# peterdavidfagan/mujoco_robot_environments

Measured on AMD Instinct MI355X. Metric: env steps/sec (whole node), RearrangementEnv batch=4096 at 1/2/4/8 MI355X, higher is better.
Workload: dtype f32

## Files before the change

### mujoco_robot_environments_amd/csrc/mre_api.cpp

```cpp
#include <hip/hip_runtime.h>

#include <cmath>
#include <cstdio>
#include <cstdlib>
#include <cstring>
#include <string>
#include <algorithm>
#include <vector>

#include "mre_env.h"
#include "mre_launch.h"
#include "mre_model.h"
#include "mre_records.h"

using namespace mre;

static thread_local std::string g_err;
int mre::fail(int code, const std::string& msg) {
  g_err = msg;
  return code;
}

extern "C" const char* mre_last_error(void) { return g_err.c_str(); }

// ... 27 lines not shown
  HIPCHK(hipMalloc(&e->sv_status, N * 4));
  HIPCHK(hipMalloc(&e->sv_converged, N));
  HIPCHK(hipHostMalloc((void**)&e->h_launch_info, mre_env::RING * N * 16, hipHostMallocMapped | hipHostMallocCoherent));
  HIPCHK(hipHostGetDevicePointer((void**)&e->d_launch_info, e->h_launch_info, 0));
  memset(e->h_launch_info, 0xFF, mre_env::RING * N * 16);
  HIPCHK(hipHostMalloc((void**)&e->h_info_last, N * 16, hipHostMallocDefault));
  memset(e->h_info_last, 0xFF, N * 16);
  HIPCHK(hipHostMalloc((void**)&e->h_large_stage, mre_env::NSTAGE * N, hipHostMallocMapped | hipHostMallocCoherent));
  HIPCHK(hipHostGetDevicePointer((void**)&e->d_large_stage, e->h_large_stage, 0));
  memset(e->h_large_stage, 0, mre_env::NSTAGE * N);
  HIPCHK(hipMalloc(&e->d_pending, N));
  HIPCHK(hipMemsetAsync(e->d_pending, 0, N, e->stream));
  HIPCHK(hipMemsetAsync(e->d_large, 0, N, e->stream));
  e->h_large.assign(N, 0); e->h_rerun.assign(N, 0);
  { int rc = sched_create(e); if (rc) return rc; }
  if (const char* fb = getenv("MRE_NO_FALLBACK")) e->fallback = atoi(fb) == 0;
  if (const char* fl = getenv("MRE_FORCE_LARGE")) {
    if (atoi(fl) != 0) {
      e->h_large.assign(N, 1); e->n_large = num_envs;
      HIPCHK(hipMemsetAsync(e->d_large, 1, N, e->stream));
    }
  }
  HIPCHK(hipMemsetAsync(e->status, 0, N * 4, e->stream)); HIPCHK(hipMemsetAsync(e->stats, 0, N * 16, e->stream));
  HIPCHK(hipMemsetAsync(e->grip_closed, 0, N, e->stream)); HIPCHK(hipMemsetAsync(e->osc_target, 0, N * 64, e->stream));
  HIPCHK(hipMemsetAsync(e->sites, 0, N * 64, e->stream));
  std::vector<int> np(N, NPROP);
  std::vector<float> ps(N * NPROP * 3, 0.0155f);
  HIPCHK(hipMemcpy(e->nprops, np.data(), N * 4, hipMemcpyHostToDevice));
  HIPCHK(hipMemcpy(e->prop_size, ps.data(), ps.size() * 4, hipMemcpyHostToDevice));
  e->osc = OscConfig{350.f, 20.f, 500.f, 100.f, 200.f, 30.f, {0.f, -0.785f, 0.f, -2.356f, 0.f, 1.571f, 0.785f},
// ... 552 lines not shown
  DRAIN(e);
  return copy_out(e, w, e->qacc_ws, (size_t)e->N * NVP * 4);
}
extern "C" int mre_set_ctrl(mre_env* e, const float* ctrl) {
  if (!e || !ctrl) return fail(MRE_ERR_ARG, "null");
  DRAIN(e);
  return copy_in(e, e->ctrl, ctrl, (size_t)e->N * NU * 4);
}

static void fill_args(mre_env* e, StepArgs& a) {
  memset(&a, 0, sizeof(a));
  a.M = e->dM; a.N = e->N; a.seq_stride = e->N;
  a.qpos = e->qpos; a.qvel = e->qvel; a.qacc_ws = e->qacc_ws; a.ctrl = e->ctrl; a.qfine = e->qfine;
  a.nprops = e->nprops; a.prop_size = e->prop_size;
  a.control_steps = 1; a.mode = CTRL_HELD;
  a.osc = e->d_osc_env ? e->d_osc_env : e->d_osc; a.osc_stride = e->d_osc_env ? 1 : 0;
  a.osc_target = e->osc_target; a.grip_closed = e->grip_closed;
  a.sites = e->sites; a.status = e->status; a.stats = e->stats; a.nstep = e->nstep;
  a.env_order = e->use_order ? e->order : (e->have_auto_order ? e->auto_order : nullptr);
  a.trace = e->trace; a.trace_nenv = e->trace_nenv; a.trace_max = e->trace_max; a.trace_base = e->trace_pos;
}

extern "C" int mre_step(mre_env* e, int nsubsteps, unsigned flags) {
  if (!e || nsubsteps < 0) return fail(MRE_ERR_ARG, "mre_step: bad argument");
  StepArgs a;
  fill_args(e, a);
  a.nsteps = nsubsteps; a.flags = flags;
  if (nsubsteps > 0) a.sites = nullptr;
  int rc = launch_step(e, a);
  if (rc) return rc;
  if (e->trace) e->trace_pos += nsubsteps;
  return MRE_OK;
}

extern "C" int mre_rollout_ticks(mre_env* e, const float* ctrl_seq, int nticks, int control_steps, unsigned flags,
                                 int ticks_per_launch) {
  if (!e || !ctrl_seq || nticks < 0 || control_steps < 1) return fail(MRE_ERR_ARG, "mre_rollout: bad argument");
  if (!is_device_ptr(ctrl_seq)) return fail(MRE_ERR_ARG, "mre_rollout: ctrl_seq must be a device pointer");
  int per = (ticks_per_launch <= 0 || ticks_per_launch > nticks) ? nticks : ticks_per_launch;
  bool allow_queue = ticks_per_launch >= 2;
  if (ticks_per_launch <= 0 && policy::queue_fits(e->queue_ok, e->queue_waves, e->N) && nticks >= 2) {
    if (policy::window_wants_queue(nticks, e->queue_min_ticks, e->tick_tail_valid, e->tick_tail, e->queue_tail_min)) {
// ... 9 lines not shown
    const size_t n = (size_t)nticks * (size_t)e->N * NU;
    if (n > e->seq_cap) {
      DRAIN_PENDING(e);
      for (float*& p : e->seq_copy) { if (p) HIPCHK(hipFree(p)); p = nullptr; HIPCHK(hipMalloc(&p, n * 4)); }
      e->seq_cap = n;
    }
    float* dst = e->seq_copy[e->seq_calls++ % (unsigned)(mre_env::RING + 1)];
    HIPCHK(hipMemcpyAsync(dst, ctrl_seq, n * 4, hipMemcpyDeviceToDevice, e->stream));
    src = dst;
  }
  for (int t0 = 0; t0 < nticks || (nticks == 0 && t0 == 0); t0 += per) {
    const int nt = nticks - t0 < per ? nticks - t0 : per;
    StepArgs a;
    fill_args(e, a);
    a.nsteps = nt * control_steps; a.control_steps = control_steps; a.mode = CTRL_SEQ;
    a.ctrl_seq = src + (size_t)t0 * (size_t)e->N * NU; a.flags = flags;
    a.sites = nullptr;
    int rc = launch_step(e, a, false, true, allow_queue);
    if (rc) return rc;
    if (e->trace) e->trace_pos += a.nsteps;
    if (nticks == 0) break;
  }
  return MRE_OK;
}

extern "C" int mre_rollout(mre_env* e, const float* ctrl_seq, int nticks, int control_steps, unsigned flags) {
  return mre_rollout_ticks(e, ctrl_seq, nticks, control_steps, flags, 0);
}

extern "C" int mre_set_trace(mre_env* e, float* out, int nenv, int max_steps) {
  if (!e) return fail(MRE_ERR_ARG, "null handle");
// ... 152 lines not shown
    if (t0 + n < nticks) a.flags |= F_CONV_OPEN;
    int rc = launch_step(e, a, false, queue || !(converged_out != nullptr && chunk >= nticks), queue);
    if (rc) return rc;
    if (e->trace) e->trace_pos += a.nsteps;
    t0 += n;
  } while (t0 < nticks);
  if (converged_out) { DRAIN(e); return copy_out(e, converged_out, e->converged, (size_t)e->N); }
  return MRE_OK;
}

extern "C" int mre_osc_compute(mre_env* e, float* tau, float* grip) {
  if (!e) return fail(MRE_ERR_ARG, "null handle");
  DRAIN(e);
  StepArgs a;
  fill_args(e, a);
  a.nsteps = 0; a.control_steps = 1; a.mode = CTRL_OSC; a.flags = F_OSC_EVAL; a.trace = nullptr;
  HIPCHK(hipSetDevice(e->device));
  step_kernels(e->solver).step(&a, e->stream);
  HIPCHK(hipGetLastError());
  const size_t N = (size_t)e->N;
  std::vector<float> h(N * NU);
  int rc = copy_out(e, h.data(), e->ctrl, N * NU * 4);
  if (rc) return rc;
  std::vector<float> ht(N * 7), hg(N);
  for (size_t i = 0; i < N; i++) {
    for (int k = 0; k < 7; k++) ht[i * 7 + k] = h[i * NU + k];
    hg[i] = h[i * NU + 7];
  }
  if (tau) { rc = copy_out(e, tau, ht.data(), N * 7 * 4); if (rc) return rc; }
  if (grip) { rc = copy_out(e, grip, hg.data(), N * 4); if (rc) return rc; }
  return MRE_OK;
// ... 9 lines not shown
  return MRE_OK;
}
static void fill_search(mre_env* e, SearchArgs& sa) {
  memset(&sa, 0, sizeof(sa));
  sa.M = e->dM; sa.N = e->N; sa.qpos = e->qpos; sa.qfine = e->qfine; sa.nprops = e->nprops; sa.prop_size = e->prop_size;
  sa.env_ids = e->d_env_ids; sa.env_id_offset = e->env_id_offset;
  sa.attempts = e->ps_attempts; sa.fixed_prop = -1;
}

static int detect_contacts(mre_env* e, const uint8_t* dmask, bool full = false, bool active_only = false) {
  const size_t N = (size_t)e->N, row = 1 + 3 * CONTACT_EXPORT;
  if (!e->contacts) HIPCHK(hipMalloc(&e->contacts, N * row * 4));
  if (full && !e->contacts_full) HIPCHK(hipMalloc(&e->contacts_full, N * CONTACT_EXPORT * 12 * 4));
  StepArgs a;
  fill_args(e, a);
  a.nsteps = 0; a.flags = F_DETECT | (active_only ? F_DETECT_ACTIVE : 0u); a.trace = nullptr; a.env_mask = dmask;
  a.contacts = e->contacts; a.contacts_full = full ? e->contacts_full : nullptr;
  a.sites = nullptr; a.geoms = nullptr;
  step_kernels(e->solver).step(&a, e->stream);
  HIPCHK(hipGetLastError());
  return MRE_OK;
}

extern "C" int mre_get_contacts(mre_env* e, int32_t* count, float* contacts) {
  if (!e || !count || !contacts) return fail(MRE_ERR_ARG, "mre_get_contacts: null");
  DRAIN(e);
  HIPCHK(hipSetDevice(e->device));
  int rc = detect_contacts(e, nullptr);
  if (rc) return rc;
  const size_t N = (size_t)e->N, row = 1 + 3 * CONTACT_EXPORT;
  std::vector<float> h(N * row);
// ... 97 lines not shown
      mre_launch_pose_search(&sa, e->stream);
      HIPCHK(hipGetLastError());
      if ((rc = copy_out(e, att.data(), e->ps_attempts, N * 4))) return rc;
      bool dropped = false;
      for (size_t i = 0; i < N; i++)
        if (todo[i] && p < np[i] && att[i] <= 0) { failed[i] = 1; todo[i] = 0; dropped = true; }
      if (dropped && (rc = copy_in(e, e->mask, todo.data(), N))) return rc;
    }
    HIPCHK(hipStreamSynchronize(e->stream));
    if (settle_steps <= 0) break;
    StepArgs a;
    fill_args(e, a);
    a.trace = nullptr;
    a.nsteps = (int)std::lround(2.0 / e->hM.opt_rec.timestep);
    if (a.nsteps < settle_steps) a.nsteps = settle_steps;
    a.flags = F_FREEZE_ROBOT | F_SETTLE_EXIT; a.env_mask = e->mask;
    a.settle_steps = e->settle_steps; a.min_settle_steps = settle_steps;
    const bool prof = e->profiling;
    e->profiling = false;
    rc = launch_step(e, a, true);
    e->profiling = prof;
    if (rc) return rc;
    if ((rc = copy_out(e, hs.data(), e->settle_steps, N * 4))) return rc;
    if (getenv("MRE_DEBUG_PLACE")) {
      int nt = 0, ns = 0;
      for (size_t i = 0; i < N; i++) if (todo[i]) { nt++; ns += hs[i] >= 0; }
      fprintf(stderr, "mre_place_props round %d: %d envs placed, %d settled\n", round, nt, ns);
    }
    int settled_now = 0;
    for (size_t i = 0; i < N; i++) {
      if (!todo[i]) continue;
// ... 159 lines not shown
```

### mujoco_robot_environments_amd/csrc/mre_collide.h

```cpp
#pragma once
#include "mre_math.h"

namespace mre {

constexpr int COLL_BUF = 48;
MRE_DEV float* cand_xyz(float* buf, int k) { return buf + 24 + 3 * k; }
MRE_DEV float& cand_dist(float* buf, int k) { return buf[3 * k + 2]; }

MRE_DEV float sel3(const float* v, int i) {
  const float w0 = i == 0 ? 1.f : 0.f, w1 = i == 1 ? 1.f : 0.f, w2 = i == 2 ? 1.f : 0.f;
  return w0 * v[0] + w1 * v[1] + w2 * v[2];
}
MRE_DEV void row3(float* o, const float (*m)[3], int i) {
  const float w0 = i == 0 ? 1.f : 0.f, w1 = i == 1 ? 1.f : 0.f, w2 = i == 2 ? 1.f : 0.f;
  o[0] = w0 * m[0][0] + w1 * m[1][0] + w2 * m[2][0];
  o[1] = w0 * m[0][1] + w1 * m[1][1] + w2 * m[2][1];
  o[2] = w0 * m[0][2] + w1 * m[1][2] + w2 * m[2][2];
}

MRE_DEV int clip_poly(float* p, float* q, int n, float sx, float sy) {
  float* src = p;
  float* dst = q;
  for (int e = 0; e < 4; e++) {
    const int ax = e >> 1;
// ... 10 lines not shown
      if (da <= 0 && nq < 8) { dst[3 * nq] = a0; dst[3 * nq + 1] = a1; dst[3 * nq + 2] = a2; nq++; }
      if ((da <= 0) != (db <= 0) && nq < 8) {
        const float t = da / (da - db);
        dst[3 * nq] = a0 + t * (b0 - a0); dst[3 * nq + 1] = a1 + t * (b1 - a1); dst[3 * nq + 2] = a2 + t * (b2 - a2);
        nq++;
      }
      a0 = b0; a1 = b1; a2 = b2;
    }
    n = nq;
    if (n == 0) return 0;
    float* t = src; src = dst; dst = t;
  }
  return n;
}

MRE_DEV int box_box(const float* p1, const float* R1, const float* s1, const float* p2,
                    const float* R2, const float* s2, float margin, float* normal, float* buf) {
  float* poly = buf;
  float* qbuf = buf + 24;
  float A[3][3], B[3][3], dv[3], Cm[3][3], aC[3][3];
#pragma unroll
  for (int i = 0; i < 3; i++)
#pragma unroll
    for (int k = 0; k < 3; k++) { A[i][k] = R1[3 * k + i]; B[i][k] = R2[3 * k + i]; }
  v3sub(dv, p2, p1);
#pragma unroll
  for (int i = 0; i < 3; i++)
#pragma unroll
    for (int j = 0; j < 3; j++) { Cm[i][j] = v3dot(A[i], B[j]); aC[i][j] = fabsf(Cm[i][j]); }
  float tA[3], tB[3];
#pragma unroll
  for (int i = 0; i < 3; i++) { tA[i] = v3dot(dv, A[i]); tB[i] = v3dot(dv, B[i]); }
  float best_face = -1e30f;
  int face_code = -1;
// ... 103 lines not shown
  v3copy(cr, pr);
  v3addscl(cr, nr, sra);
#pragma unroll
  for (int v = 0; v < 4; v++) {
    const float su = (v == 0 || v == 3) ? 1.0f : -1.0f;
    const float sv = (v < 2) ? 1.0f : -1.0f;
    float w[3];
    v3copy(w, ci);
    v3addscl(w, Aiu, su * siu);
    v3addscl(w, Aiv, sv * siv);
    v3sub(w, w, cr);
    poly[3 * v] = v3dot(w, Aru);
    poly[3 * v + 1] = v3dot(w, Arv);
    poly[3 * v + 2] = v3dot(w, nr);
  }
  const int n = clip_poly(poly, qbuf, 4, sru, srv);
  int nc = 0;
  for (int v = 0; v < n; v++) {
    const float x = poly[3 * v], y = poly[3 * v + 1], dep = poly[3 * v + 2];
    if (dep > margin) continue;
    float* cx = cand_xyz(buf, nc);
    cx[0] = cr[0] + x * Aru[0] + y * Arv[0] + 0.5f * dep * nr[0];
    cx[1] = cr[1] + x * Aru[1] + y * Arv[1] + 0.5f * dep * nr[1];
    cx[2] = cr[2] + x * Aru[2] + y * Arv[2] + 0.5f * dep * nr[2];
    cand_dist(buf, nc) = dep;
    nc++;
  }
  return nc;
}

MRE_DEV int plane_box(const float* pp, const float* Rp, const float* pb, const float* Rb,
                      const float* sb, float margin, float* normal, float* buf) {
  float n[3] = {Rp[2], Rp[5], Rp[8]};
  v3copy(normal, n);
  int cnt = 0;
  for (int c = 0; c < 8 && cnt < 4; c++) {
    float loc[3] = {(c & 1) ? sb[0] : -sb[0], (c & 2) ? sb[1] : -sb[1], (c & 4) ? sb[2] : -sb[2]};
    float w[3], wd[3];
    m3mulv(w, Rb, loc);
    if (v3dot(w, n) > 0.f) continue;
    v3add(w, w, pb);
    v3sub(wd, w, pp);
    const float ds = v3dot(wd, n);
// ... 119 lines not shown
```

### mujoco_robot_environments_amd/csrc/mre_dev.h

```cpp
#pragma once
#include <stdint.h>

namespace mre {

constexpr int NB = 20;
constexpr int NRB = 16;
constexpr int GRIP_BODY0 = 8;
constexpr int NV = 39;
constexpr int NRV = 15;
constexpr int NQ = 43;
constexpr int NQP = 44;
constexpr int TRACE_W = 88;
constexpr int TRACE_QVEL = 48;
constexpr int NVP = 40;
constexpr int NU = 8;
constexpr int QFINE = 32;
constexpr int QFINE_ROW = 96;
constexpr int QFINE_CUBE_Q = 32;
constexpr int QFINE_CUBE_V = 60;
static_assert(QFINE_CUBE_Q + 7 * 4 == QFINE_CUBE_V && QFINE_CUBE_V + 6 * 4 <= QFINE_ROW, "qfine row layout");
constexpr int NPROP = 4;
constexpr int NG = 20;
constexpr int PROP_GEOM0 = 12;
constexpr int NPAIR = 128;
// ... 138 lines not shown
  MEntryRec m_rec[NMR];
  RowRec row_rec[NROWREC];
  EqRec eq_rec[NEQ];
  SiteRec site_rec[NSITE];
  OptRec opt_rec;
};

struct OscConfig {
  float kp_pos, kd_pos, kp_ori, kd_ori, kp_null, kd_null;
  float null_q[7];
  float pos_thresh, ori_thresh;
  int pinv_always;
};

enum StepFlags : unsigned { F_NO_CONSTRAINTS = 1u, F_FREEZE_ROBOT = 2u, F_CONV_CONTINUE = 4u, F_CONV_OPEN = 8u,
                            F_OSC_EVAL = 16u, F_DETECT = 32u, F_SETTLE_EXIT = 64u, F_DETECT_ACTIVE = 128u };
enum CtrlMode : int { CTRL_HELD = 0, CTRL_SEQ = 1, CTRL_OSC = 2 };

struct StepArgs {
  const DevModel* M;
  int N;
  float* qpos;
  float* qvel;
  float* qacc_ws;
  float* qfine;
  float* ctrl;
  const float* ctrl_seq;
  int seq_stride;
  const int* nprops;
  const float* prop_size;
  int nsteps, control_steps, mode;
// ... 121 lines not shown
```

### mujoco_robot_environments_amd/csrc/mre_env.h

```cpp
#pragma once
#include <hip/hip_runtime.h>

#include <string>
#include <utility>
#include <vector>

#include "../../include/mre.h"
#include "mre_dev.h"
#include "mre_policy.h"

#define HIPCHK(x)                                                                       \
  do {                                                                                  \
    hipError_t e_ = (x);                                                                \
    if (e_ != hipSuccess)                                                               \
      return mre::fail(MRE_ERR_HIP, std::string(#x) + ": " + hipGetErrorString(e_));    \
  } while (0)

struct mre_env {
  int N = 0, device = 0;
  hipStream_t stream = nullptr;
  mre::DevModel* dM = nullptr;
  mre::DevModel hM;
  int solver = MRE_SOLVER_PGS;
  float *qpos = nullptr, *qvel = nullptr, *qacc_ws = nullptr, *ctrl = nullptr;
// ... 66 lines not shown
    int head = 0, nout = 0;
    int cur = 0;
    int* h_order = nullptr;
    int* d_order = nullptr;
  };
  std::vector<Group> groups;
  int* h_grp_order = nullptr;
  int* d_grp_order = nullptr;
  Group qgroup;
  bool queue_ok = true;
  int queue_ticks = 200;
  int queue_waves = 0;
  int queue_shards = 16;
  int queue_lshards = 8;
  bool queue_test_serial = false;
  int queue_spare_large = 8;
  int queue_run_ticks = 100;
  int queue_min_ticks = 32;
  float tick_tail = 0.f;
  bool tick_tail_valid = false;
  float queue_tail_min = 1.45f;
  unsigned tail_samples = 0;
  std::vector<int> tail_scratch;
  int queue_large_waves_max = 0;
  int* h_qlist = nullptr;
  int* q_ws = nullptr;
  int* q_gen = nullptr;
  int* h_q_err = nullptr;
  int* h_qgrp_order = nullptr;
  long n_queue_launches = 0;
// ... 37 lines not shown
```

### mujoco_robot_environments_amd/csrc/mre_kernels.hip

```cpp
#include <hip/hip_runtime.h>

#include "mre_dev.h"
#include "mre_math.h"
#include "mre_collide.h"

namespace mre {
using ModelP = MRE_MODEL_PTR(DevModel);
#if defined(MRE_PHASE_STAMPS) && MRE_PHASE_STAMPS >= 4
__shared__ unsigned long long dbg_acc[4];
#endif

struct OscSm {
  float J[6][7], M[7][7], MiJt[7][6], Li[6][6], Lam[6][6], V[6][6], Jbar[7][6];
  float ep[3], eo[3], F[6], LF[6], tn[7], Jbt[6], xd[6], w[6];
};

struct alignas(8) Blk {
  uint16_t row0;
  uint8_t type, nrows;
  uint8_t rslot;
  uint8_t pa, pb;
  uint8_t primary : 4;
  uint8_t bslot : 4;
};
// ... 1382 lines not shown
    crb_mass_matrix(M, s, l);
    MRE_SYNC();
#ifndef MRE_NEWTON
    factor_robot_regs(s.qM, s.qLD, s.qLDinv);
#endif
    MRE_STAMP(15);
    MRE_STAMP(0);

    velocity_stage(M, s, l);
    MRE_SYNC();
    finger_bias(M, s, l);
    MRE_STAMP(1);
    const bool constrained = (a.flags & F_NO_CONSTRAINTS) == 0;
    if (constrained) {

      collide(M, s, l, false);
      MRE_STAMP(2);
      assemble_constraints(M, s, l);
#ifdef MRE_NEWTON
      nw_build_lists(s, l);
#else
      solve_robot_rows(s, l);
      assemble_blocks(M, s, l);
#endif
      MRE_STAMP(3);
      hw_ncon = max(hw_ncon, s.ncon); hw_nefc = max(hw_nefc, s.nefc);
      hw_nrrow = max(hw_nrrow, s.nrrow); hw_npp = max(hw_npp, s.npp);
    }

    if (a.mode == CTRL_SEQ && (step % a.control_steps) == 0) {
      const int tick = step / a.control_steps;
// ... 85 lines not shown
    else a.nstep[env] += steps_done;
  }
  if (a.nsteps == 0 && (a.flags & F_OSC_EVAL) != 0 && a.mode == CTRL_OSC) {
    position_stage(M, s, l);
    gripper_local(M, s, l);
    crb_mass_matrix(M, s, l);
    MRE_SYNC();
    velocity_stage(M, s, l);
    MRE_SYNC();
    osc_compute(M, s, osc, oscp, s.osc_tgt, l);
    if (l == 0) s.ctrl[NU - 1] = grip_cmd;
    MRE_SYNC();
  }
  if (a.nsteps == 0 && (a.flags & F_DETECT) != 0 && a.contacts != nullptr) {
    position_stage(M, s, l);
    collide(M, s, l, (a.flags & F_DETECT_ACTIVE) == 0);
    float* o = a.contacts + (size_t)env * (1 + 3 * CONTACT_EXPORT);
    const int n = s.ncon < CONTACT_EXPORT ? s.ncon : CONTACT_EXPORT;
    if (l == 0) o[0] = s.overflow ? -(float)s.ncon : (float)s.ncon;
    if (l < n) {
      const int pr = s.con_pair[l];
      o[1 + 3 * l] = (float)M->pair_g1[pr]; o[2 + 3 * l] = (float)M->pair_g2[pr]; o[3 + 3 * l] = s.con_dist[l];
      if (a.contacts_full != nullptr) {
        float* f = a.contacts_full + ((size_t)env * CONTACT_EXPORT + l) * 12;
        for (int k = 0; k < 3; k++) f[k] = s.con_pos[l][k];
        for (int k = 0; k < 9; k++) f[3 + k] = s.con_frame[l][k];
      }
    }
    MRE_SYNC();
    if (l == 0) s.overflow = 0;
  }
// ... 485 lines not shown
```

### mujoco_robot_environments_amd/csrc/mre_math.h

```cpp
#pragma once
#include <hip/hip_runtime.h>

#define MRE_DEV __device__ __forceinline__
#if defined(MRE_PHASE_STAMPS) && MRE_PHASE_STAMPS >= 4
#define MRE_DBG_T0() unsigned long long dbg_t_ = __builtin_amdgcn_s_memtime()
#define MRE_DBG_STAMP(SET, K)                                                      \
  do {                                                                             \
    const unsigned long long n_ = __builtin_amdgcn_s_memtime();                    \
    if (MRE_PHASE_STAMPS == (SET) && threadIdx.x == 0) dbg_acc[K] += n_ - dbg_t_;  \
    dbg_t_ = n_;                                                                   \
  } while (0)
#else
#define MRE_DBG_T0() do {} while (0)
#define MRE_DBG_STAMP(SET, K) do {} while (0)
#endif
#define MRE_PHASE_FN __device__ __attribute__((noinline))
#define MRE_SYNC()                                        \
  do {                                                    \
    __builtin_amdgcn_fence(__ATOMIC_ACQ_REL, "wavefront"); \
    __builtin_amdgcn_wave_barrier();                      \
  } while (0)
#if defined(__HIP_DEVICE_COMPILE__)
#define MRE_MODEL_PTR(T) const T __attribute__((address_space(1)))*
#else
#define MRE_MODEL_PTR(T) const T*
#endif

namespace mre {

constexpr float kMinVal = 1e-15f;

MRE_DEV void keep_live(float x) { asm volatile("" ::"v"(x)); }
MRE_DEV void keep_live(int x) { asm volatile("" ::"v"(x)); }

MRE_DEV void v3copy(float* r, const float* a) { r[0] = a[0]; r[1] = a[1]; r[2] = a[2]; }
MRE_DEV void v3zero(float* r) { r[0] = r[1] = r[2] = 0.f; }
MRE_DEV void v3add(float* r, const float* a, const float* b) {
  r[0] = a[0] + b[0]; r[1] = a[1] + b[1]; r[2] = a[2] + b[2];
}
MRE_DEV void v3sub(float* r, const float* a, const float* b) {
  r[0] = a[0] - b[0]; r[1] = a[1] - b[1]; r[2] = a[2] - b[2];
}
MRE_DEV float v3dot(const float* a, const float* b) { return a[0] * b[0] + a[1] * b[1] + a[2] * b[2]; }
MRE_DEV void v3cross(float* r, const float* a, const float* b) {
  float x = a[1] * b[2] - a[2] * b[1], y = a[2] * b[0] - a[0] * b[2], z = a[0] * b[1] - a[1] * b[0];
  r[0] = x; r[1] = y; r[2] = z;
}
MRE_DEV void v3addscl(float* r, const float* a, float s) { r[0] += a[0] * s; r[1] += a[1] * s; r[2] += a[2] * s; }
// ... 176 lines not shown
```

### mujoco_robot_environments_amd/csrc/mre_solver.h

```cpp
#pragma once

namespace mre {

constexpr int HDR_NONE = 0xFF;
constexpr int BLK_NONE = 0x7F;
constexpr int SCHED_NONE = 0xFF;
constexpr int TAB_OFF = MAXBLK * 5;
constexpr int TAB_ZEROS = 48;
static_assert(TAB_BYTES == 8 * (TAB_OFF + 1) + 4 * TAB_ZEROS, "operand table size");

#ifndef MRE_NEWTON
MRE_DEV void build_schedule(ModelP M, Sm& s);
#endif
MRE_DEV constexpr int cube_pair_bit(int p, int q) {
  const int a = p < q ? p : q, b = p < q ? q : p;
  return a == 0 ? b - 1 : (a == 1 ? b + 1 : 5);
}

MRE_DEV float prop_invM(const Sm& s, int p, int k) {
  return 1.0f / ((k < 3) ? s.prop_mass[p] : s.prop_inertia[p][k - 3]);
}

MRE_DEV void geom_pose(ModelP M, const Sm& s, int g, float* p, float* R, float* size,
                       float* rbound) {
// ... 10 lines not shown
  } else {
    v3copy(size, M->geom_size[g]);
    *rbound = M->geom_rbound[g];
  }
}

MRE_DEV void geom_center(ModelP M, const Sm& s, int g, float* p, float* rbound) {
  const int b = M->geom_body[g];
  float tmp[3];
  m3mulv(tmp, s.xmat[b], M->geom_pos[g]);
  v3add(p, s.xpos[b], tmp);
  const int pid = M->geom_propid[g];
  *rbound = pid >= 0 ? v3norm(s.prop_size[pid]) : M->geom_rbound[g];
}

MRE_PHASE_FN void collide(ModelP M, Sm& s, int l, bool detect) {
  static_assert(offsetof(Sm, hdr) + sizeof(((Sm*)0)->hdr) - offsetof(Sm, JpA) >= sizeof(float) * 64 * COLL_BUF,
                "clip buffers do not fit");
  static_assert(NPAIR <= 256 && sizeof(((Sm*)0)->iscr) >= NPAIR, "survivor list: one byte per pair");
  MRE_DBG_T0();
  float* buf = &s.JpA[0][0] + l * COLL_BUF;
  uint8_t* list = reinterpret_cast<uint8_t*>(s.iscr);
  const unsigned long long lt = (1ull << l) - 1ull;
  int nsurv = 0;
  for (int pass = 0; pass < NPAIR / 64; pass++) {
    const int pr = l + 64 * pass;
    const auto* R = &M->pair_rec[pr];
    const int g1 = R->g1, b1 = R->b1, b2 = R->b2, pid1 = R->pid1, pid2 = R->pid2, type1 = R->type1;
    const float lp1[3] = {R->pos1[0], R->pos1[1], R->pos1[2]}, lp2[3] = {R->pos2[0], R->pos2[1], R->pos2[2]};
    const float mrb1 = R->rb1, mrb2 = R->rb2, margin = R->margin, gap = R->gap;
    const float lq1[4] = {R->quat1[0], R->quat1[1], R->quat1[2], R->quat1[3]};
// ... 89 lines not shown
      cand_dist(buf, 0) = dmin;
    }
    if (n > 0) {
      float f[9];
      v3copy(f, normal);
      make_frame(f);
      for (int c = 0; c < n; c++) {
        const int id = off + c;
        if (id >= NCON_MAX) break;
        const float cx0 = cand_xyz(buf, c)[0], cx1 = cand_xyz(buf, c)[1], cx2 = cand_xyz(buf, c)[2];
        s.con_pos[id][0] = cx0; s.con_pos[id][1] = cx1; s.con_pos[id][2] = cx2;
        for (int k = 0; k < 9; k++) s.con_frame[id][k] = f[k];
        s.con_dist[id] = cand_dist(buf, c);
        s.con_pair[id] = (uint8_t)pr;
      }
    }
    MRE_SYNC();
    MRE_DBG_STAMP(6, 3);
    if (tot > NCON_MAX) break;
    base = tot;
  }
}

MRE_DEV float impedance(const float* solimp, float pos, float margin) {
  const float dmin = clampf(solimp[0], 0.0001f, 0.9999f), dmax = clampf(solimp[1], 0.0001f, 0.9999f);
  const float width = fmaxf(solimp[2], kMinVal), mid = clampf(solimp[3], 0.0001f, 0.9999f);
  const float power = fmaxf(solimp[4], 1.0f);
  if (dmin == dmax) return 0.5f * (dmin + dmax);
  const float x = fabsf((pos - margin) / width);
  if (x >= 1.0f) return dmax;
// ... 860 lines not shown
```

Baseline: 23.96 million.

## Parallelize box-box face clipping across lanes and lane-parallel contact write-out

Box-box narrowphase now defers polygon clipping to a job record, and groups of 8 lanes cooperatively clip each job with ballot/popcount compaction instead of one lane running the serial clip loop. Contact frame write-out is also redistributed so each lane handles one contact via a contact map, instead of per-pair serial loops. This targets warp divergence from a few lanes doing long clipping work. In exchange it adds extra syncs and shared-buffer traffic. The old path is kept behind an environment flag.

```diff
diff --git a/mujoco_robot_environments_amd/csrc/mre_api.cpp b/mujoco_robot_environments_amd/csrc/mre_api.cpp
--- a/mujoco_robot_environments_amd/csrc/mre_api.cpp
+++ b/mujoco_robot_environments_amd/csrc/mre_api.cpp
@@ -65,6 +65,7 @@
   HIPCHK(hipMemsetAsync(e->d_large, 0, N, e->stream));
   e->h_large.assign(N, 0); e->h_rerun.assign(N, 0);
   { int rc = sched_create(e); if (rc) return rc; }
+  if (const char* cs = getenv("MRE_COLLIDE_SERIAL")) e->base_flags = atoi(cs) != 0 ? F_COLLIDE_SERIAL : 0u;
   if (const char* fb = getenv("MRE_NO_FALLBACK")) e->fallback = atoi(fb) == 0;
   if (const char* fl = getenv("MRE_FORCE_LARGE")) {
     if (atoi(fl) != 0) {
@@ -647,6 +648,7 @@
   a.qpos = e->qpos; a.qvel = e->qvel; a.qacc_ws = e->qacc_ws; a.ctrl = e->ctrl; a.qfine = e->qfine;
   a.nprops = e->nprops; a.prop_size = e->prop_size;
   a.control_steps = 1; a.mode = CTRL_HELD;
+  a.flags = e->base_flags;
   a.osc = e->d_osc_env ? e->d_osc_env : e->d_osc; a.osc_stride = e->d_osc_env ? 1 : 0;
   a.osc_target = e->osc_target; a.grip_closed = e->grip_closed;
   a.sites = e->sites; a.status = e->status; a.stats = e->stats; a.nstep = e->nstep;
@@ -658,7 +660,7 @@
   if (!e || nsubsteps < 0) return fail(MRE_ERR_ARG, "mre_step: bad argument");
   StepArgs a;
   fill_args(e, a);
-  a.nsteps = nsubsteps; a.flags = flags;
+  a.nsteps = nsubsteps; a.flags |= flags;
   if (nsubsteps > 0) a.sites = nullptr;
   int rc = launch_step(e, a);
   if (rc) return rc;
@@ -698,7 +700,7 @@
     StepArgs a;
     fill_args(e, a);
     a.nsteps = nt * control_steps; a.control_steps = control_steps; a.mode = CTRL_SEQ;
-    a.ctrl_seq = src + (size_t)t0 * (size_t)e->N * NU; a.flags = flags;
+    a.ctrl_seq = src + (size_t)t0 * (size_t)e->N * NU; a.flags |= flags;
     a.sites = nullptr;
     int rc = launch_step(e, a, false, true, allow_queue);
     if (rc) return rc;
@@ -881,7 +883,7 @@
   DRAIN(e);
   StepArgs a;
   fill_args(e, a);
-  a.nsteps = 0; a.control_steps = 1; a.mode = CTRL_OSC; a.flags = F_OSC_EVAL; a.trace = nullptr;
+  a.nsteps = 0; a.control_steps = 1; a.mode = CTRL_OSC; a.flags |= F_OSC_EVAL; a.trace = nullptr;
   HIPCHK(hipSetDevice(e->device));
   step_kernels(e->solver).step(&a, e->stream);
   HIPCHK(hipGetLastError());
@@ -921,7 +923,7 @@
   if (full && !e->contacts_full) HIPCHK(hipMalloc(&e->contacts_full, N * CONTACT_EXPORT * 12 * 4));
   StepArgs a;
   fill_args(e, a);
-  a.nsteps = 0; a.flags = F_DETECT | (active_only ? F_DETECT_ACTIVE : 0u); a.trace = nullptr; a.env_mask = dmask;
+  a.nsteps = 0; a.flags |= F_DETECT | (active_only ? F_DETECT_ACTIVE : 0u); a.trace = nullptr; a.env_mask = dmask;
   a.contacts = e->contacts; a.contacts_full = full ? e->contacts_full : nullptr;
   a.sites = nullptr; a.geoms = nullptr;
   step_kernels(e->solver).step(&a, e->stream);
@@ -1049,7 +1051,7 @@
     a.trace = nullptr;
     a.nsteps = (int)std::lround(2.0 / e->hM.opt_rec.timestep);
     if (a.nsteps < settle_steps) a.nsteps = settle_steps;
-    a.flags = F_FREEZE_ROBOT | F_SETTLE_EXIT; a.env_mask = e->mask;
+    a.flags |= F_FREEZE_ROBOT | F_SETTLE_EXIT; a.env_mask = e->mask;
     a.settle_steps = e->settle_steps; a.min_settle_steps = settle_steps;
     const bool prof = e->profiling;
     e->profiling = false;
diff --git a/mujoco_robot_environments_amd/csrc/mre_collide.h b/mujoco_robot_environments_amd/csrc/mre_collide.h
--- a/mujoco_robot_environments_amd/csrc/mre_collide.h
+++ b/mujoco_robot_environments_amd/csrc/mre_collide.h
@@ -48,10 +48,15 @@
   return n;
 }
 
-MRE_DEV int box_box(const float* p1, const float* R1, const float* s1, const float* p2,
-                    const float* R2, const float* s2, float margin, float* normal, float* buf) {
+struct FaceJob { float cr[3], Aru[3], Arv[3], nr[3], sru, srv; };
+constexpr int JOB_PARAM = 24, JOB_WORDS = 15;
+static_assert(JOB_PARAM >= 12 && JOB_PARAM + JOB_WORDS <= COLL_BUF, "job record: inside the pair's clip buffer, behind the quad");
+static_assert(sizeof(FaceJob) == 4 * (JOB_WORDS - 1), "job record: FaceJob and the margin");
+
+template <bool JOB>
+MRE_DEV int box_box_impl(const float* p1, const float* R1, const float* s1, const float* p2,
+                         const float* R2, const float* s2, float margin, float* normal, float* buf) {
   float* poly = buf;
-  float* qbuf = buf + 24;
   float A[3][3], B[3][3], dv[3], Cm[3][3], aC[3][3];
 #pragma unroll
   for (int i = 0; i < 3; i++)
@@ -185,19 +190,92 @@
     poly[3 * v + 1] = v3dot(w, Arv);
     poly[3 * v + 2] = v3dot(w, nr);
   }
-  const int n = clip_poly(poly, qbuf, 4, sru, srv);
-  int nc = 0;
-  for (int v = 0; v < n; v++) {
-    const float x = poly[3 * v], y = poly[3 * v + 1], dep = poly[3 * v + 2];
-    if (dep > margin) continue;
-    float* cx = cand_xyz(buf, nc);
-    cx[0] = cr[0] + x * Aru[0] + y * Arv[0] + 0.5f * dep * nr[0];
-    cx[1] = cr[1] + x * Aru[1] + y * Arv[1] + 0.5f * dep * nr[1];
-    cx[2] = cr[2] + x * Aru[2] + y * Arv[2] + 0.5f * dep * nr[2];
-    cand_dist(buf, nc) = dep;
-    nc++;
-  }
-  return nc;
+  if constexpr (JOB) {
+    float* o = buf + JOB_PARAM;
+#pragma unroll
+    for (int k = 0; k < 3; k++) { o[k] = cr[k]; o[3 + k] = Aru[k]; o[6 + k] = Arv[k]; o[9 + k] = nr[k]; }
+    o[12] = sru; o[13] = srv; o[14] = margin;
+    return -1;
+  } else {
+    float* qbuf = buf + 24;
+    const int n = clip_poly(poly, qbuf, 4, sru, srv);
+    int nc = 0;
+    for (int v = 0; v < n; v++) {
+      const float x = poly[3 * v], y = poly[3 * v + 1], dep = poly[3 * v + 2];
+      if (dep > margin) continue;
+      float* cx = cand_xyz(buf, nc);
+      cx[0] = cr[0] + x * Aru[0] + y * Arv[0] + 0.5f * dep * nr[0];
+      cx[1] = cr[1] + x * Aru[1] + y * Arv[1] + 0.5f * dep * nr[1];
+      cx[2] = cr[2] + x * Aru[2] + y * Arv[2] + 0.5f * dep * nr[2];
+      cand_dist(buf, nc) = dep;
+      nc++;
+    }
+    return nc;
+  }
+}
+MRE_DEV int box_box(const float* p1, const float* R1, const float* s1, const float* p2,
+                    const float* R2, const float* s2, float margin, float* normal, float* buf) {
+  return box_box_impl<false>(p1, R1, s1, p2, R2, s2, margin, normal, buf);
+}
+
+MRE_DEV void job_load(const float* buf, FaceJob& J, float& margin) {
+  const float* o = buf + JOB_PARAM;
+#pragma unroll
+  for (int k = 0; k < 3; k++) { J.cr[k] = o[k]; J.Aru[k] = o[3 + k]; J.Arv[k] = o[6 + k]; J.nr[k] = o[9 + k]; }
+  J.sru = o[12]; J.srv = o[13]; margin = o[14];
+}
+MRE_DEV void clip_lane(const float* src, int n, int i, int e, float sx, float sy, bool& keep, bool& cross, float* a, float* x) {
+  const int ax = e >> 1;
+  const float sg = (e & 1) ? -1.0f : 1.0f;
+  const float lim = ax ? sy : sx;
+  keep = false; cross = false;
+  a[0] = a[1] = a[2] = 0.f; x[0] = x[1] = x[2] = 0.f;
+  if (i < n) {
+    const int i2 = i + 1 == n ? 0 : i + 1;
+    const float a0 = src[3 * i], a1 = src[3 * i + 1], a2 = src[3 * i + 2];
+    const float b0 = src[3 * i2], b1 = src[3 * i2 + 1], b2 = src[3 * i2 + 2];
+    const float da = sg * (ax ? a1 : a0) - lim, db = sg * (ax ? b1 : b0) - lim;
+    keep = da <= 0;
+    cross = (da <= 0) != (db <= 0);
+    a[0] = a0; a[1] = a1; a[2] = a2;
+    if (cross) {
+      const float t = da / (da - db);
+      x[0] = a0 + t * (b0 - a0); x[1] = a1 + t * (b1 - a1); x[2] = a2 + t * (b2 - a2);
+    }
+  }
+}
+MRE_DEV int clip_slot(unsigned kb, unsigned cb, int i) {
+  const unsigned lo = (1u << i) - 1u;
+  return __builtin_popcount(kb & lo) + __builtin_popcount(cb & lo);
+}
+MRE_DEV int clip_count(unsigned kb, unsigned cb) {
+  const int t = __builtin_popcount(kb) + __builtin_popcount(cb);
+  return t < 8 ? t : 8;
+}
+MRE_DEV void clip_lane_store(float* dst, int slot, bool keep, bool cross, const float* a, const float* x) {
+  if (keep && slot < 8) { dst[3 * slot] = a[0]; dst[3 * slot + 1] = a[1]; dst[3 * slot + 2] = a[2]; }
+  const int sx = slot + (keep ? 1 : 0);
+  if (cross && sx < 8) { dst[3 * sx] = x[0]; dst[3 * sx + 1] = x[1]; dst[3 * sx + 2] = x[2]; }
+}
+MRE_DEV void cand_lane(const float* poly, int n, int i, const FaceJob& J, float margin, bool& keep, float* cx, float& dep) {
+  keep = false; dep = 0.f;
+  cx[0] = cx[1] = cx[2] = 0.f;
+  if (i < n) {
+    const float x = poly[3 * i], y = poly[3 * i + 1];
+    dep = poly[3 * i + 2];
+    keep = !(dep > margin) && dep < margin;
+    cx[0] = J.cr[0] + x * J.Aru[0] + y * J.Arv[0] + 0.5f * dep * J.nr[0];
+    cx[1] = J.cr[1] + x * J.Aru[1] + y * J.Arv[1] + 0.5f * dep * J.nr[1];
+    cx[2] = J.cr[2] + x * J.Aru[2] + y * J.Arv[2] + 0.5f * dep * J.nr[2];
+  }
+}
+MRE_DEV void cand_lane_store(float* buf, unsigned kb, int i, bool keep, const float* cx, float dep) {
+  if (keep) {
+    const int slot = __builtin_popcount(kb & ((1u << i) - 1u));
+    float* o = cand_xyz(buf, slot);
+    o[0] = cx[0]; o[1] = cx[1]; o[2] = cx[2];
+    cand_dist(buf, slot) = dep;
+  }
 }
 
 MRE_DEV int plane_box(const float* pp, const float* Rp, const float* pb, const float* Rb,
diff --git a/mujoco_robot_environments_amd/csrc/mre_dev.h b/mujoco_robot_environments_amd/csrc/mre_dev.h
--- a/mujoco_robot_environments_amd/csrc/mre_dev.h
+++ b/mujoco_robot_environments_amd/csrc/mre_dev.h
@@ -176,7 +176,8 @@
 };
 
 enum StepFlags : unsigned { F_NO_CONSTRAINTS = 1u, F_FREEZE_ROBOT = 2u, F_CONV_CONTINUE = 4u, F_CONV_OPEN = 8u,
-                            F_OSC_EVAL = 16u, F_DETECT = 32u, F_SETTLE_EXIT = 64u, F_DETECT_ACTIVE = 128u };
+                            F_OSC_EVAL = 16u, F_DETECT = 32u, F_SETTLE_EXIT = 64u, F_DETECT_ACTIVE = 128u,
+                            F_COLLIDE_SERIAL = 256u };
 enum CtrlMode : int { CTRL_HELD = 0, CTRL_SEQ = 1, CTRL_OSC = 2 };
 
 struct StepArgs {
diff --git a/mujoco_robot_environments_amd/csrc/mre_env.h b/mujoco_robot_environments_amd/csrc/mre_env.h
--- a/mujoco_robot_environments_amd/csrc/mre_env.h
+++ b/mujoco_robot_environments_amd/csrc/mre_env.h
@@ -104,6 +104,7 @@
   int queue_shards = 16;
   int queue_lshards = 8;
   bool queue_test_serial = false;
+  unsigned base_flags = 0;
   int queue_spare_large = 8;
   int queue_run_ticks = 100;
   int queue_min_ticks = 32;
diff --git a/mujoco_robot_environments_amd/csrc/mre_kernels.hip b/mujoco_robot_environments_amd/csrc/mre_kernels.hip
--- a/mujoco_robot_environments_amd/csrc/mre_kernels.hip
+++ b/mujoco_robot_environments_amd/csrc/mre_kernels.hip
@@ -1420,7 +1420,8 @@
     const bool constrained = (a.flags & F_NO_CONSTRAINTS) == 0;
     if (constrained) {
 
-      collide(M, s, l, false);
+      if ((a.flags & F_COLLIDE_SERIAL) != 0) collide_serial(M, s, l, false);
+      else collide(M, s, l, false);
       MRE_STAMP(2);
       assemble_constraints(M, s, l);
 #ifdef MRE_NEWTON
@@ -1536,7 +1537,8 @@
   }
   if (a.nsteps == 0 && (a.flags & F_DETECT) != 0 && a.contacts != nullptr) {
     position_stage(M, s, l);
-    collide(M, s, l, (a.flags & F_DETECT_ACTIVE) == 0);
+    if ((a.flags & F_COLLIDE_SERIAL) != 0) collide_serial(M, s, l, (a.flags & F_DETECT_ACTIVE) == 0);
+    else collide(M, s, l, (a.flags & F_DETECT_ACTIVE) == 0);
     float* o = a.contacts + (size_t)env * (1 + 3 * CONTACT_EXPORT);
     const int n = s.ncon < CONTACT_EXPORT ? s.ncon : CONTACT_EXPORT;
     if (l == 0) o[0] = s.overflow ? -(float)s.ncon : (float)s.ncon;
diff --git a/mujoco_robot_environments_amd/csrc/mre_math.h b/mujoco_robot_environments_amd/csrc/mre_math.h
--- a/mujoco_robot_environments_amd/csrc/mre_math.h
+++ b/mujoco_robot_environments_amd/csrc/mre_math.h
@@ -1,7 +1,9 @@
 #pragma once
 #include <hip/hip_runtime.h>
 
+#ifndef MRE_DEV
 #define MRE_DEV __device__ __forceinline__
+#endif
 #if defined(MRE_PHASE_STAMPS) && MRE_PHASE_STAMPS >= 4
 #define MRE_DBG_T0() unsigned long long dbg_t_ = __builtin_amdgcn_s_memtime()
 #define MRE_DBG_STAMP(SET, K)                                                      \
@@ -32,6 +34,7 @@
 
 MRE_DEV void keep_live(float x) { asm volatile("" ::"v"(x)); }
 MRE_DEV void keep_live(int x) { asm volatile("" ::"v"(x)); }
+MRE_DEV int opaque(int x) { asm volatile("" : "+v"(x)); return x; }
 
 MRE_DEV void v3copy(float* r, const float* a) { r[0] = a[0]; r[1] = a[1]; r[2] = a[2]; }
 MRE_DEV void v3zero(float* r) { r[0] = r[1] = r[2] = 0.f; }
diff --git a/mujoco_robot_environments_amd/csrc/mre_solver.h b/mujoco_robot_environments_amd/csrc/mre_solver.h
--- a/mujoco_robot_environments_amd/csrc/mre_solver.h
+++ b/mujoco_robot_environments_amd/csrc/mre_solver.h
@@ -48,7 +48,7 @@
   *rbound = pid >= 0 ? v3norm(s.prop_size[pid]) : M->geom_rbound[g];
 }
 
-MRE_PHASE_FN void collide(ModelP M, Sm& s, int l, bool detect) {
+MRE_PHASE_FN void collide_serial(ModelP M, Sm& s, int l, bool detect) {
   static_assert(offsetof(Sm, hdr) + sizeof(((Sm*)0)->hdr) - offsetof(Sm, JpA) >= sizeof(float) * 64 * COLL_BUF,
                 "clip buffers do not fit");
   static_assert(NPAIR <= 256 && sizeof(((Sm*)0)->iscr) >= NPAIR, "survivor list: one byte per pair");
@@ -168,6 +168,202 @@
         s.con_dist[id] = cand_dist(buf, c);
         s.con_pair[id] = (uint8_t)pr;
       }
+    }
+    MRE_SYNC();
+    MRE_DBG_STAMP(6, 3);
+    if (tot > NCON_MAX) break;
+    base = tot;
+  }
+}
+
+constexpr int JOB_COUNT = 6;
+MRE_DEV void clip_job_lanes(float* jbuf, bool valid, int l) {
+  const int i = l & 7, sh = l & 56;
+  FaceJob J = {};
+  float margin = 0.f;
+  if (valid) job_load(jbuf, J, margin);
+  MRE_SYNC();
+  int n = valid ? 4 : 0;
+  float* src = jbuf;
+  float* dst = jbuf + 24;
+#pragma unroll
+  for (int e = 0; e < 4; e++) {
+    bool keep, cross;
+    float a[3], x[3];
+    clip_lane(src, n, i, e, J.sru, J.srv, keep, cross, a, x);
+    const unsigned kb = (unsigned)(__ballot(keep) >> sh) & 0xFFu, cb = (unsigned)(__ballot(cross) >> sh) & 0xFFu;
+    clip_lane_store(dst, clip_slot(kb, cb, i), keep, cross, a, x);
+    n = clip_count(kb, cb);
+    MRE_SYNC();
+    float* t = src; src = dst; dst = t;
+  }
+  bool keep;
+  float cx[3], dep;
+  cand_lane(src, n, i, J, margin, keep, cx, dep);
+  const unsigned kb = (unsigned)(__ballot(keep) >> sh) & 0xFFu;
+  MRE_SYNC();
+  cand_lane_store(jbuf, kb, i, keep, cx, dep);
+  if (valid && i == 0) reinterpret_cast<int*>(jbuf)[JOB_COUNT] = __builtin_popcount(kb);
+}
+
+MRE_PHASE_FN void collide(ModelP M, Sm& s, int l, bool detect) {
+  static_assert(offsetof(Sm, hdr) + sizeof(((Sm*)0)->hdr) - offsetof(Sm, JpA) >= sizeof(float) * 64 * COLL_BUF,
+                "clip buffers do not fit");
+  static_assert(NPAIR == 128 && sizeof(((Sm*)0)->iscr) >= NPAIR + 2 * 64 && NCON_MAX <= 64,
+                "survivor list: one byte per pair; behind it the contact map: 16 bits per contact, one lane per contact");
+  MRE_DBG_T0();
+  float* buf0 = &s.JpA[0][0];
+  uint8_t* list = reinterpret_cast<uint8_t*>(s.iscr);
+  uint16_t* cmap = reinterpret_cast<uint16_t*>(list + NPAIR);
+  const unsigned long long lt = (1ull << l) - 1ull;
+  int nsurv = 0;
+  for (int pass = 0; pass < NPAIR / 64; pass++) {
+    const int pr = l + 64 * pass;
+    const auto* R = &M->pair_rec[pr];
+    const int g1 = R->g1, b1 = R->b1, b2 = R->b2, pid1 = R->pid1, pid2 = R->pid2, type1 = R->type1;
+    const float lp1[3] = {R->pos1[0], R->pos1[1], R->pos1[2]}, lp2[3] = {R->pos2[0], R->pos2[1], R->pos2[2]};
+    const float mrb1 = R->rb1, mrb2 = R->rb2, margin = R->margin, gap = R->gap;
+    const float lq1[4] = {R->quat1[0], R->quat1[1], R->quat1[2], R->quat1[3]};
+    bool live = false;
+    if (g1 >= 0 && (pid1 < 0 || pid1 < s.nprops) && (pid2 < 0 || pid2 < s.nprops)) {
+      const float inc = detect ? margin : margin - gap;
+      float p1[3], p2[3], df[3], tmp[3];
+      m3mulv(tmp, s.xmat[b1], lp1); v3add(p1, s.xpos[b1], tmp);
+      m3mulv(tmp, s.xmat[b2], lp2); v3add(p2, s.xpos[b2], tmp);
+      const float rb1 = pid1 >= 0 ? v3norm(s.prop_size[pid1]) : mrb1, rb2 = pid2 >= 0 ? v3norm(s.prop_size[pid2]) : mrb2;
+      v3sub(df, p2, p1);
+      if (type1 == 0) {
+        float q[4], R1[9];
+        qmul(q, s.xquat[b1], lq1);
+        q2mat(R1, q);
+        const float nn[3] = {R1[2], R1[5], R1[8]};
+        live = v3dot(df, nn) - rb2 <= inc;
+      } else {
+        const float r = rb1 + rb2 + inc;
+        live = v3dot(df, df) <= r * r;
+      }
+    }
+    const unsigned long long m = __ballot(live);
+    if (live) list[nsurv + __popcll(m & lt)] = (uint8_t)pr;
+    nsurv += __popcll(m);
+  }
+  if (l == 0) s.ncon = 0;
+  MRE_SYNC();
+  MRE_DBG_STAMP(6, 0);
+  int base = 0;
+  for (int c0 = 0; c0 < nsurv; c0 += 64) {
+    const int pr = (c0 + l < nsurv) ? list[c0 + l] : -1;
+    float normal[3] = {0.f, 0.f, 1.f};
+    int n = 0;
+    bool isjob = false;
+    float* buf = buf0 + opaque(l) * COLL_BUF;
+    int rsingle = 0;
+    float margin = 0.f, gap = 0.f;
+    if (pr >= 0) {
+      const auto* R = &M->pair_rec[pr];
+      const int b1 = R->b1, b2 = R->b2, pid1 = R->pid1, pid2 = R->pid2, type1 = R->type1;
+      rsingle = R->single;
+      const float lp1[3] = {R->pos1[0], R->pos1[1], R->pos1[2]}, lp2[3] = {R->pos2[0], R->pos2[1], R->pos2[2]};
+      const float lq1[4] = {R->quat1[0], R->quat1[1], R->quat1[2], R->quat1[3]};
+      const float lq2[4] = {R->quat2[0], R->quat2[1], R->quat2[2], R->quat2[3]};
+      const float ms1[3] = {R->size1[0], R->size1[1], R->size1[2]}, ms2[3] = {R->size2[0], R->size2[1], R->size2[2]};
+      margin = R->margin; gap = R->gap;
+      float p1[3], R1[9], s1[3], p2[3], R2[9], s2[3], tmp[3], q[4];
+      m3mulv(tmp, s.xmat[b1], lp1); v3add(p1, s.xpos[b1], tmp);
+      qmul(q, s.xquat[b1], lq1); q2mat(R1, q);
+      m3mulv(tmp, s.xmat[b2], lp2); v3add(p2, s.xpos[b2], tmp);
+      qmul(q, s.xquat[b2], lq2); q2mat(R2, q);
+      if (pid1 >= 0) v3copy(s1, s.prop_size[pid1]); else v3copy(s1, ms1);
+      if (pid2 >= 0) v3copy(s2, s.prop_size[pid2]); else v3copy(s2, ms2);
+      const float inc = detect ? margin : margin - gap;
+      MRE_DBG_STAMP(6, 1);
+      if ((rsingle >> 8) == 2) n = cyl_box(p1, R1, s1, p2, R2, s2[0], s2[2], inc, normal, buf);
+      else if (type1 == 0) n = plane_box(p1, R1, p2, R2, s2, inc, normal, buf);
+      else {
+        n = box_box_impl<true>(p1, R1, s1, p2, R2, s2, inc, normal, buf);
+        if (n < 0) { isjob = true; n = 0; }
+      }
+      int m = 0;
+      for (int c = 0; c < n; c++)
+        if (cand_dist(buf, c) < inc) {
+          if (m != c) {
+            for (int k = 0; k < 3; k++) cand_xyz(buf, m)[k] = cand_xyz(buf, c)[k];
+            cand_dist(buf, m) = cand_dist(buf, c);
+          }
+          m++;
+        }
+      n = m;
+    }
+    MRE_SYNC();
+    const int lb = opaque(l);
+    buf = buf0 + lb * COLL_BUF;
+    {
+      unsigned long long jm = __ballot(isjob);
+      const int g = lb >> 3;
+      while (jm) {
+        int jl = -1;
+#pragma unroll
+        for (int k = 0; k < 8; k++) {
+          const int ln = __ffsll((long long)jm) - 1;
+          if (g == k) jl = ln;
+          jm &= jm - 1ull;
+        }
+        clip_job_lanes(buf0 + (jl >= 0 ? jl : lb) * COLL_BUF, jl >= 0, lb);
+        MRE_SYNC();
+      }
+      if (isjob) n = reinterpret_cast<const int*>(buf)[JOB_COUNT];
+    }
+    MRE_DBG_STAMP(6, 2);
+    const bool single = pr >= 0 && n > 1 && (rsingle & 0xFF) != 0;
+    const int ncand = n;
+    if (single) n = 1;
+    int off = base, tot = base;
+    for (int bit = 0; bit < 4; bit++) {
+      const unsigned long long m = __ballot((n >> bit) & 1);
+      off += __popcll(m & lt) << bit;
+      tot += __popcll(m) << bit;
+    }
+    const int lim = tot < NCON_MAX ? tot : NCON_MAX;
+    if (l == 0) {
+      s.ncon = lim;
+      if (tot > NCON_MAX) s.overflow = 1;
+    }
+    if (single) {
+      const float incw = margin - gap;
+      float wsum = 0.f, px = 0.f, py = 0.f, pz = 0.f, dmin = cand_dist(buf, 0);
+      int best = 0;
+      for (int c = 0; c < ncand; c++) {
+        const float dc = cand_dist(buf, c);
+        if (dc < dmin) { dmin = dc; best = c; }
+        const float w = incw - dc;
+        if (w > 0.f) { wsum += w; px += w * cand_xyz(buf, c)[0]; py += w * cand_xyz(buf, c)[1]; pz += w * cand_xyz(buf, c)[2]; }
+      }
+      if (wsum > 0.f) { const float iw = 1.0f / wsum; px *= iw; py *= iw; pz *= iw; }
+      else { px = cand_xyz(buf, best)[0]; py = cand_xyz(buf, best)[1]; pz = cand_xyz(buf, best)[2]; }
+      cand_xyz(buf, 0)[0] = px; cand_xyz(buf, 0)[1] = py; cand_xyz(buf, 0)[2] = pz;
+      cand_dist(buf, 0) = dmin;
+    }
+    if (n > 0) {
+#pragma unroll
+      for (int c = 0; c < 8; c++)
+        if (c < n && off + c < NCON_MAX) cmap[off + c] = (uint16_t)(lb << 3 | c);
+      buf[0] = normal[0]; buf[1] = normal[1]; buf[3] = normal[2];
+      reinterpret_cast<int*>(buf)[4] = pr;
+    }
+    MRE_SYNC();
+    if (lb >= base && lb < lim) {
+      const int src = cmap[lb], c = src & 7;
+      const float* sb = buf0 + (src >> 3) * COLL_BUF;
+      float f[9];
+      f[0] = sb[0]; f[1] = sb[1]; f[2] = sb[3];
+      const int spr = reinterpret_cast<const int*>(sb)[4];
+      const float cx0 = sb[24 + 3 * c], cx1 = sb[24 + 3 * c + 1], cx2 = sb[24 + 3 * c + 2];
+      const float dist = sb[3 * c + 2];
+      make_frame(f);
+      s.con_pos[lb][0] = cx0; s.con_pos[lb][1] = cx1; s.con_pos[lb][2] = cx2;
+      for (int k = 0; k < 9; k++) s.con_frame[lb][k] = f[k];
+      s.con_dist[lb] = dist;
+      s.con_pair[lb] = (uint8_t)spr;
     }
     MRE_SYNC();
     MRE_DBG_STAMP(6, 3);
```

Measured after the change: 24.85 million, median of 5. 1.04x the previous value.
